# weitong8591/differentiable_ransac

Hardware: AMD Instinct MI355X
Metric: hypotheses/sec (and image-pairs/sec) at 2000 pts x 1024 hyps, 1/2/4/8 GPU (higher is better)
Workload: dtype f32; 1 GPU; nister 5-pt E, 2000 pts x 1024 hyps per pair, Gumbel top-k sampler (in-kernel Philox), MSAC scoring with masks, test mode, 128 pairs/GPU/step; sampler=gumbel, pairs_per_gpu=128, points=2000, hypotheses_per_pair=1024, hypotheses_per_pair_per_gpu=1024, models_per_pair=10240, solver=nister, parallelism=pairs sharded over 1 GPU(s), no collective, streams=1, issue=1 batch(es) in flight, round-robin over 1 HIP stream(s), eager launches

## Files before the change

differentiable_ransac_amd/csrc/dr_common.hpp:

```cpp
#pragma once
#include <hip/hip_runtime.h>
#include <stdint.h>
#include <stdio.h>

#include "../../include/dransac.h"

namespace dr {

constexpr int kWave = 64;

void set_error(const char *fmt, ...);

inline int check_launch(const char *what) {
  hipError_t e = hipGetLastError();
  if (e != hipSuccess) {
    set_error("%s: %s", what, hipGetErrorString(e));
    return DR_ELAUNCH;
  }
  return DR_OK;
}

#define DR_REQUIRE(cond, msg)            \
  do {                                   \
    if (!(cond)) {                       \
      ::dr::set_error("%s: %s", __func__, msg); \
      return DR_EINVAL;                  \
    }                                    \
  } while (0)

struct PairGate {
  const int32_t *iters = nullptr;
  const double *max_iters = nullptr;
  __device__ __forceinline__ bool closed(int p) const { return iters && (double)iters[p] >= max_iters[p]; }
  __device__ __forceinline__ bool closed_range(int first, int last) const {
    if (!iters) return false;
    for (int p = first; p <= last; ++p)
      if (!closed(p)) return false;
    return true;
  }
};

__device__ __forceinline__ void seed_next_block(uint64_t *__restrict__ state, uint64_t *__restrict__ out, int n) {
  const uint64_t s0 = state[0] * 0x9E3779B97F4A7C15ull + state[1];
  for (int i = threadIdx.x; i < n; i += blockDim.x) out[i] = s0 + (uint64_t)i;
  __syncthreads();
  if (threadIdx.x == 0) state[1] += (uint64_t)n;
}

__device__ __forceinline__ void race_weights_block(const float *__restrict__ logits, int N, int P, int p, float *__restrict__ ws) {
  __shared__ float s_mx[4], s_mn[4], s_rate[4];
  __shared__ int s_bad[4];
  const int tid = threadIdx.x, lane = tid & 63, wv = tid >> 6;
  const float *lg = logits + (size_t)p * N;
  constexpr int kRegs = 8;
  const bool in_regs = N <= kRegs * 256;
  float lr[kRegs];
  float mx = -INFINITY, mn = INFINITY;
  int bad = 0;
  if (in_regs) {
#pragma unroll
    for (int u = 0; u < kRegs; ++u) lr[u] = (tid + 256 * u < N) ? lg[tid + 256 * u] : 0.f;
#pragma unroll
    for (int u = 0; u < kRegs; ++u) {
      const bool have = tid + 256 * u < N, fin = fabsf(lr[u]) < INFINITY;
      bad |= (have && !fin) ? 1 : 0;
      mx = (have && fin) ? fmaxf(mx, lr[u]) : mx;
      mn = (have && fin) ? fminf(mn, lr[u]) : mn;
    }
  } else {
    for (int n = tid; n < N; n += 256) {
      const float l = lg[n];
      const bool fin = fabsf(l) < INFINITY;
      bad |= fin ? 0 : 1;
      mx = fin ? fmaxf(mx, l) : mx;
      mn = fin ? fminf(mn, l) : mn;
    }
  }
#pragma unroll
  for (int o = 32; o > 0; o >>= 1) {
    mx = fmaxf(mx, __shfl_xor(mx, o, 64));
    mn = fminf(mn, __shfl_xor(mn, o, 64));
    bad |= __shfl_xor(bad, o, 64);
  }
  if (lane == 0) { s_mx[wv] = mx; s_mn[wv] = mn; s_bad[wv] = bad; }
  __syncthreads();
  mx = fmaxf(fmaxf(s_mx[0], s_mx[1]), fmaxf(s_mx[2], s_mx[3]));
  mn = fminf(fminf(s_mn[0], s_mn[1]), fminf(s_mn[2], s_mn[3]));
  bad = s_bad[0] | s_bad[1] | s_bad[2] | s_bad[3];
  const bool tame = !bad && (mx - mn) <= 80.0f;
  float *w = ws + (size_t)p * N;
  float rate = 0.f;
  if (in_regs) {
#pragma unroll
    for (int u = 0; u < kRegs; ++u) {
      if (tid + 256 * u < N) {
        const float d = (mx - lr[u]) * 1.44269504088896340736f;
        w[tid + 256 * u] = tame ? __builtin_amdgcn_exp2f(d) : 0.f;
        rate += tame ? __builtin_amdgcn_exp2f(-d) : 0.f;
      }
    }
  } else {
    for (int n = tid; n < N; n += 256) {
      const float d = (mx - lg[n]) * 1.44269504088896340736f;
      w[n] = tame ? __builtin_amdgcn_exp2f(d) : 0.f;
      rate += tame ? __builtin_amdgcn_exp2f(-d) : 0.f;
    }
  }
#pragma unroll
  for (int o = 32; o > 0; o >>= 1) rate += __shfl_xor(rate, o, 64);
  if (lane == 0) s_rate[wv] = rate;
  __syncthreads();
  if (tid == 0) {
    reinterpret_cast<int *>(ws + (size_t)P * N)[p] = tame ? 1 : 0;
    ws[(size_t)P * N + P + p] = -1.0f / (0.69314718055994530942f * ((s_rate[0] + s_rate[1]) + (s_rate[2] + s_rate[3])));
    ws[(size_t)P * N + 2 * (size_t)P + p] = mx;
  }
}

template <typename T>
__device__ __forceinline__ T wave_sum(T v) {
#pragma unroll
  for (int o = 32; o > 0; o >>= 1) v += __shfl_xor(v, o, 64);
  return v;
}
__device__ __forceinline__ float wave_sum_lane63(float v) {
  v += __int_as_float(__builtin_amdgcn_mov_dpp(__float_as_int(v), 0xB1, 0xF, 0xF, true));
  v += __int_as_float(__builtin_amdgcn_mov_dpp(__float_as_int(v), 0x4E, 0xF, 0xF, true));
  v += __int_as_float(__builtin_amdgcn_mov_dpp(__float_as_int(v), 0x141, 0xF, 0xF, true));
  v += __int_as_float(__builtin_amdgcn_mov_dpp(__float_as_int(v), 0x140, 0xF, 0xF, true));
  v += __int_as_float(__builtin_amdgcn_update_dpp(0, __float_as_int(v), 0x142, 0xA, 0xF, false));
  v += __int_as_float(__builtin_amdgcn_update_dpp(0, __float_as_int(v), 0x143, 0xC, 0xF, false));
  return v;
}

template <int kCtrl, int kRowMask, bool kBound>
__device__ __forceinline__ double dpp_add_step(double x) {
  const long long xi = __double_as_longlong(x);
  const int lo = (int)xi, hi = (int)(xi >> 32);
  const int tlo = kBound ? __builtin_amdgcn_mov_dpp(lo, kCtrl, kRowMask, 0xF, true) : __builtin_amdgcn_update_dpp(0, lo, kCtrl, kRowMask, 0xF, false);
  const int thi = kBound ? __builtin_amdgcn_mov_dpp(hi, kCtrl, kRowMask, 0xF, true) : __builtin_amdgcn_update_dpp(0, hi, kCtrl, kRowMask, 0xF, false);
  return x + __longlong_as_double(((long long)thi << 32) | (unsigned int)tlo);
}
__device__ __forceinline__ double wave_sum_lane63(double v) {
  v = dpp_add_step<0xB1, 0xF, true>(v);
  v = dpp_add_step<0x4E, 0xF, true>(v);
  v = dpp_add_step<0x141, 0xF, true>(v);
  v = dpp_add_step<0x140, 0xF, true>(v);
  v = dpp_add_step<0x142, 0xA, false>(v);
  v = dpp_add_step<0x143, 0xC, false>(v);
  return v;
}

template <int kCtrl, int kRowMask>
__device__ __forceinline__ float dpp_max_step(float x) {
  const int xi = __float_as_int(x);
  return fmaxf(x, __int_as_float(__builtin_amdgcn_update_dpp(xi, xi, kCtrl, kRowMask, 0xF, false)));
}
__device__ __forceinline__ float wave_max_bcast(float v) {
  v = dpp_max_step<0xB1, 0xF>(v);
  v = dpp_max_step<0x4E, 0xF>(v);
  v = dpp_max_step<0x141, 0xF>(v);
  v = dpp_max_step<0x140, 0xF>(v);
  v = dpp_max_step<0x142, 0xA>(v);
  v = dpp_max_step<0x143, 0xC>(v);
  return __int_as_float(__builtin_amdgcn_readlane(__float_as_int(v), 63));
}
__device__ __forceinline__ float wave_sum_bcast(float v) {
  return __int_as_float(__builtin_amdgcn_readlane(__float_as_int(wave_sum_lane63(v)), 63));
}

template <typename T>
__device__ __forceinline__ T wave_max(T v) {
#pragma unroll
  for (int o = 32; o > 0; o >>= 1) {
    T w = __shfl_xor(v, o, 64);
    v = w > v ? w : v;
  }
  return v;
}

__device__ __forceinline__ float fast_rcp(float x) { return __builtin_amdgcn_rcpf(x); }
__device__ __forceinline__ double fast_rcp(double x) { return 1.0 / x; }

template <typename T>
__device__ __forceinline__ bool is_finite(T x) {
  return __builtin_isfinite(x);
}

struct Philox {
  static constexpr uint32_t M0 = 0xD2511F53u, M1 = 0xCD9E8D57u, W0 = 0x9E3779B9u, W1 = 0xBB67AE85u;
  __host__ __device__ static inline void mulhilo(uint32_t a, uint32_t b, uint32_t &hi, uint32_t &lo) {
    uint64_t p = (uint64_t)a * b;
    hi = (uint32_t)(p >> 32);
    lo = (uint32_t)p;
  }
  __host__ __device__ static inline uint32_t xor3(uint32_t a, uint32_t b, uint32_t c) {
#if defined(__HIP_DEVICE_COMPILE__)
    uint32_t r;
    asm("v_bitop3_b32 %0, %1, %2, %3 bitop3:0x96" : "=v"(r) : "v"(a), "v"(b), "s"(c));
    return r;
#else
    return a ^ b ^ c;
#endif
  }
  __host__ __device__ static inline void gen(uint64_t seed, uint32_t c0, uint32_t c1, uint32_t c2, uint32_t c3,
                                             uint32_t out[4]) {
    uint32_t k0 = (uint32_t)seed, k1 = (uint32_t)(seed >> 32);
    constexpr int kPhiloxRounds = 7;
#pragma unroll
    for (int r = 0; r < kPhiloxRounds; ++r) {
      uint32_t h0, l0, h1, l1;
      mulhilo(M0, c0, h0, l0);
      mulhilo(M1, c2, h1, l1);
      uint32_t n0 = xor3(h1, c1, k0), n1 = l1, n2 = xor3(h0, c3, k1), n3 = l0;
      c0 = n0; c1 = n1; c2 = n2; c3 = n3;
      k0 += W0; k1 += W1;
    }
    out[0] = c0; out[1] = c1; out[2] = c2; out[3] = c3;
  }
};

__device__ __forceinline__ float gumbel_from_bits(uint32_t bits) {
  constexpr float kScale = 2.3283064365386963e-10f * (1.0f - 1.1920928955078125e-07f - 1.17549435e-38f);
  float u = __builtin_fmaf((float)bits, kScale, 1.17549435e-38f);
  const float kLn2 = 0.69314718055994530942f;
  const float t = __builtin_amdgcn_logf(u);
  float g = __builtin_fmaf(-kLn2, __builtin_amdgcn_logf(-t), 0.36651292058166432701f);
  asm("" : "+v"(g));
  return g;
}

#ifdef DR_PROFILE_STAGES
static __device__ unsigned long long g_stage_cycles[32];
#define DR_STAGE_BEGIN() unsigned long long _t_prev = __builtin_readcyclecounter()
#define DR_STAGE(i)                                                        \
  do {                                                                     \
    unsigned long long _t = __builtin_readcyclecounter();                  \
    if ((threadIdx.x & 63) == 0) atomicAdd(&::dr::g_stage_cycles[i], _t - _t_prev); \
    _t_prev = __builtin_readcyclecounter();                                \
  } while (0)
#define DR_DEFINE_STAGE_READER(name)                                                                          \
  extern "C" int name(unsigned long long *out16) {                                            \
    unsigned long long zero[32] = {0};                                                                        \
    if (hipMemcpyFromSymbol(out16, HIP_SYMBOL(::dr::g_stage_cycles), sizeof(zero)) != hipSuccess) return -2; \
    if (hipMemcpyToSymbol(HIP_SYMBOL(::dr::g_stage_cycles), zero, sizeof(zero)) != hipSuccess) return -2;    \
    return 0;                                                                                                 \
  }
#else
#define DR_DEFINE_STAGE_READER(name)
#define DR_STAGE_BEGIN() do {} while (0)
#define DR_STAGE(i) do {} while (0)
#endif

}
```

differentiable_ransac_amd/csrc/gumbel_topk.hip:

```cpp
#include <algorithm>

#include "dr_common.hpp"

namespace dr {

constexpr int kRowsPerBlock = 4;
constexpr int kMaxK = 8;
constexpr int kMaxCand = 64;

template <typename T>
struct GumbelArgs {
  const T *logits;
  const T *gumbel;
  uint64_t seed;
  T tau;
  int P, B, N, k;
  const uint64_t *seed_ptr;
  int sub;
};
__device__ __forceinline__ void sub_batch_row(uint64_t &seed, int &bq, int b, int sub) {
  bq = b;
  if (sub > 0) {
    seed += (uint64_t)(b / sub);
    bq = b % sub;
// ... 204 lines not shown
      if (kSoft) y_sel[row * a.k + pos] = exp_t<T>(mg - wmx) * inv_sm;
      s_win[wv][pos] = me;
    }
  }
  if (kSoft && lane == 0) lse_out[row] = lse;

  if (kSoft && (y_soft || ret)) {
    __builtin_amdgcn_fence(__ATOMIC_ACQ_REL, "workgroup");
    __builtin_amdgcn_wave_barrier();
    int mine[kMaxK];
    for (int r = 0; r < kMaxK; ++r) mine[r] = r < a.k ? winp[r] : -1;
    for (int q = lane; q < groups; q += 64) {
      T g[4];
      if (kCache) {
#pragma unroll
        for (int j = 0; j < 4; ++j) g[j] = gcache[4 * q + j];
      } else {
        T nz[4];
        load_group<T>(a, p, b, q, g, nz);
      }
#pragma unroll
      for (int j = 0; j < 4; ++j) {
        const int n = 4 * q + j;
        if (n >= a.N) continue;
        const T y = exp_t<T>(g[j] - wmx) * inv_sm;
        bool sel = false;
#pragma unroll
        for (int r = 0; r < kMaxK; ++r) sel = sel || (mine[r] == n);
        if (y_soft) y_soft[row * a.N + n] = y;
        if (ret) ret[row * a.N + n] = ((sel ? T(1) : T(0)) - y) + y;
      }
    }
  }
}

__device__ __forceinline__ float log2_uniform_from_bits(uint32_t bits) {
  constexpr float kScale = 2.3283064365386963e-10f * (1.0f - 1.1920928955078125e-07f - 1.17549435e-38f);
  return __builtin_amdgcn_logf(__builtin_fmaf((float)bits, kScale, 1.17549435e-38f));
}

__global__ __launch_bounds__(256) void gumbel_race_weights_kernel(const float *__restrict__ logits, int N, int P, float *__restrict__ ws) {
  race_weights_block(logits, N, P, blockIdx.x, ws);
}

constexpr int kFastGroups = 8;

__device__ __forceinline__ float4 straight_through(float4 m, float y) {
  const float st = (1.0f - y) + y;
  return make_float4(m.x * st, m.y * st, m.z * st, m.w * st);
}

template <bool kSoft, bool kScreen = false>
__global__ __launch_bounds__(kRowsPerBlock * 64) void gumbel_topk_fast_kernel(const float *__restrict__ logits, uint64_t seed,
                                                                             int B, int N, int k, int32_t *__restrict__ idx,
                                                                             float *__restrict__ y_sel,
                                                                             float *__restrict__ lse_out,
                                                                             const uint64_t *__restrict__ seed_ptr,
                                                                             const float4 *__restrict__ gather_src = nullptr,
                                                                             float4 *__restrict__ gather_dst = nullptr,
                                                                             PairGate gate = PairGate(),
                                                                             const uint32_t *__restrict__ screen_tb = nullptr,
                                                                             const float *__restrict__ screen_T = nullptr,
                                                                             int sub = 0, const float *__restrict__ race_ws = nullptr,
                                                                             int P_race = 0) {
  if (gate.closed(blockIdx.y)) return;
  static_assert(!(kSoft && kScreen), "the soft-max statistics need every element's score");
  __shared__ float s_val[kRowsPerBlock][kMaxCand];
  __shared__ int s_idx[kRowsPerBlock][kMaxCand];
  if (seed_ptr) seed = *seed_ptr;
  const int lane = threadIdx.x & 63;
  int wv = threadIdx.x >> 6;
  wv = __builtin_amdgcn_readfirstlane(wv);
  const int p = blockIdx.y, b = blockIdx.x * kRowsPerBlock + wv;
  if (b >= B) return;
  int bq;
  sub_batch_row(seed, bq, b, sub);
  const int groups = N >> 2;
  const size_t row = (size_t)p * B + b;
  const float4 *lg = reinterpret_cast<const float4 *>(logits + (size_t)p * N);
  float *cand_val = s_val[wv];
  int *cand_idx = s_idx[wv];

  if constexpr (kScreen) {
    const float Tf = screen_T[p];
    if (Tf != INFINITY) {
      const uint4 *tb4 = reinterpret_cast<const uint4 *>(screen_tb + (size_t)p * N);
      int ncand = 0, reach = 0;
      uint4 t_nx = lane < groups ? tb4[lane] : make_uint4(0xffffffffu, 0xffffffffu, 0xffffffffu, 0xffffffffu);
      float4 l_nx = lane < groups ? lg[lane] : make_float4(0.f, 0.f, 0.f, 0.f);
#pragma unroll
      for (int i = 0; i < kFastGroups; ++i) {
        if (64 * i >= groups) break;
        const int q = lane + 64 * i;
        const bool inb = q < groups;
        const uint4 t4 = t_nx;
        const float4 l4v = l_nx;
        if (i + 1 < kFastGroups) {
          const int qn = q + 64;
          t_nx = qn < groups ? tb4[qn] : make_uint4(0xffffffffu, 0xffffffffu, 0xffffffffu, 0xffffffffu);
          l_nx = qn < groups ? lg[qn] : make_float4(0.f, 0.f, 0.f, 0.f);
        }
        uint32_t r[4];
        Philox::gen(seed, (uint32_t)q, (uint32_t)bq, (uint32_t)p, 0u, r);
        const uint32_t tt[4] = {t4.x, t4.y, t4.z, t4.w};
        const float ll[4] = {l4v.x, l4v.y, l4v.z, l4v.w};
#pragma unroll
        for (int j = 0; j < 4; ++j) {
          const bool has = inb && r[j] >= tt[j];
          const unsigned long long bal = __builtin_amdgcn_ballot_w64(has);
          if (bal) {
            float gv = -INFINITY;
            if (has) {
              gv = ll[j] + gumbel_from_bits(r[j]);
              const int pos = ncand + __popcll(bal & ((1ull << lane) - 1ull));
              if (pos < kMaxCand) { cand_val[pos] = gv; cand_idx[pos] = 4 * q + j; }
            }
            ncand += __popcll(bal);
            reach += __popcll(__builtin_amdgcn_ballot_w64(has && gv >= Tf));
          }
        }
      }
      __builtin_amdgcn_fence(__ATOMIC_ACQ_REL, "workgroup");
      __builtin_amdgcn_wave_barrier();
      if (reach >= k && ncand <= kMaxCand) {
        const bool have = lane < ncand;
        const float cv = have ? cand_val[lane] : -INFINITY;
        const int ci = have ? cand_idx[lane] : 0x7fffffff;
        int rank = 0;
        for (int j = 0; j < ncand; ++j) {
          const float ov = cand_val[j];
          const int oi = cand_idx[j];
          rank += (ov > cv) || (ov == cv && oi < ci);
        }
        const bool win = have && rank < k;
        const unsigned long long wb = __ballot(win);
        int pos = 0;
        for (int j = 0; j < ncand; ++j) {
          if ((wb >> j) & 1ull) pos += cand_idx[j] < ci;
        }
        if (win) {
          idx[row * k + pos] = ci;
          if (gather_dst) gather_dst[row * k + pos] = gather_src[(size_t)p * N + ci];
        }
        return;
      }
      __builtin_amdgcn_wave_barrier();
    }
  }

  float g[kFastGroups][4];
  float mx = -INFINITY, sm = 0.f, lmax = -INFINITY;
  bool race = false;
  if constexpr (!kScreen) race = race_ws != nullptr && reinterpret_cast<const int *>(race_ws + (size_t)P_race * N)[p] != 0;
  if (race) {
    const float4 *wr = reinterpret_cast<const float4 *>(race_ws + (size_t)p * N);
#pragma unroll
    for (int i = 0; i < kFastGroups; ++i) {
      const int q = lane + 64 * i;
      if (q < groups) {
        uint32_t r[4];
        Philox::gen(seed, (uint32_t)q, (uint32_t)bq, (uint32_t)p, 0u, r);
        const float4 w4 = wr[q];
        g[i][0] = w4.x * log2_uniform_from_bits(r[0]);
        g[i][1] = w4.y * log2_uniform_from_bits(r[1]);
        g[i][2] = w4.z * log2_uniform_from_bits(r[2]);
        g[i][3] = w4.w * log2_uniform_from_bits(r[3]);
        lmax = fmaxf(lmax, fmaxf(fmaxf(g[i][0], g[i][1]), fmaxf(g[i][2], g[i][3])));
        if (kSoft) sm += (__builtin_amdgcn_rcpf(-g[i][0]) + __builtin_amdgcn_rcpf(-g[i][1])) +
                         (__builtin_amdgcn_rcpf(-g[i][2]) + __builtin_amdgcn_rcpf(-g[i][3]));
      } else {
#pragma unroll
        for (int j = 0; j < 4; ++j) g[i][j] = -INFINITY;
      }
    }
  } else
#pragma unroll
  for (int i = 0; i < kFastGroups; ++i) {
    const int q = lane + 64 * i;
    if (q < groups) {
      uint32_t r[4];
      Philox::gen(seed, (uint32_t)q, (uint32_t)bq, (uint32_t)p, 0u, r);
      const float4 l = lg[q];
      g[i][0] = l.x + gumbel_from_bits(r[0]);
      g[i][1] = l.y + gumbel_from_bits(r[1]);
      g[i][2] = l.z + gumbel_from_bits(r[2]);
      g[i][3] = l.w + gumbel_from_bits(r[3]);
      const float gm = fmaxf(fmaxf(g[i][0], g[i][1]), fmaxf(g[i][2], g[i][3]));
      lmax = fmaxf(lmax, gm);
      if (kSoft) {
        if (gm > mx) { sm *= exp_t<float>(mx - gm); mx = gm; }
#pragma unroll
        for (int j = 0; j < 4; ++j) sm += exp_t<float>(g[i][j] - mx);
      }
    } else {
#pragma unroll
      for (int j = 0; j < 4; ++j) g[i][j] = -INFINITY;
    }
  }
  float wmx = 0.f, lse = 0.f, inv_sm = 0.f;
  if (kSoft) {
    if (race) {
      sm = row_sum(sm);
      lse = race_ws[(size_t)P_race * N + 2 * (size_t)P_race + p] + (log_t<float>(sm) + 0.36651292058166432701f);
      inv_sm = 1.0f / sm;
    } else {
      wmx = row_max(mx);
      sm *= (mx == -INFINITY) ? 0.f : exp_t<float>(mx - wmx);
      sm = row_sum(sm);
      lse = wmx + log_t<float>(sm);
      inv_sm = 1.0f / sm;
    }
  }
  auto y_of = [&](float score) { return race ? __builtin_amdgcn_rcpf(-score) * inv_sm : exp_t<float>(score - wmx) * inv_sm; };

  bool settled = false;
  float thr = -INFINITY;
  if constexpr (!kScreen) if (race) {
    const float inv = race_ws[(size_t)P_race * N + P_race + p];
    const float kf = (float)k + 0.5f;
    float t = 6.0f * inv, tlo = 0.f, thi = 0.f;
    int clo = 0;
    bool have_lo = false, have_hi = false;
#pragma unroll
    for (int it = 0; it < 6; ++it) {
      const int c = __popcll(__builtin_amdgcn_ballot_w64(lmax >= t));
      if (c >= k) { tlo = t; clo = c; have_lo = true; if (c == k) break; }
      else { thi = t; have_hi = true; }
      t = (have_lo && have_hi) ? 0.5f * (tlo + thi) : t * fminf(4.0f, kf * __builtin_amdgcn_rcpf((float)c + 0.5f));
    }
    if (have_lo && clo <= 16) { settled = true; thr = tlo; }
  }
  if (!settled) {
    float v = lmax;
    for (int r = 0; r < k; ++r) {
      thr = row_max(v);
      const unsigned long long who = __ballot(v == thr);
      if (lane == __ffsll((long long)who) - 1) v = -INFINITY;
    }
  }

  if constexpr (!kScreen) {
    int n = 0;
    int cv_i = __float_as_int(-INFINITY), ci = 0x7fffffff;
#pragma unroll
    for (int i = 0; i < kFastGroups; ++i) {
      if (64 * i >= groups) break;
      const unsigned long long c0 = __builtin_amdgcn_ballot_w64(g[i][0] >= thr), c1 = __builtin_amdgcn_ballot_w64(g[i][1] >= thr),
                               c2 = __builtin_amdgcn_ballot_w64(g[i][2] >= thr), c3 = __builtin_amdgcn_ballot_w64(g[i][3] >= thr);
      unsigned long long any = c0 | c1 | c2 | c3;
      while (any) {
        const int l = __builtin_ctzll(any);
        any &= any - 1;
        const unsigned long long cj[4] = {c0, c1, c2, c3};
#pragma unroll
        for (int j = 0; j < 4; ++j) {
          if ((cj[j] >> l) & 1ull) {
            const bool mine = __builtin_amdgcn_inverse_ballot_w64(1ull << (n & 63));
            cv_i = mine ? __builtin_amdgcn_readlane(__float_as_int(g[i][j]), l) : cv_i;
            ci = mine ? 4 * (l + 64 * i) + j : ci;
            ++n;
          }
        }
      }
    }
    if (n <= 64) {
      const float cv = __int_as_float(cv_i);
      bool win = lane < n;
      int pos = lane;
      if (n > k) {
        int rank = 0;
#pragma unroll 1
        for (int m = 0; m < n; ++m) {
          const float ov = __int_as_float(__builtin_amdgcn_readlane(cv_i, m));
          const int oi = __builtin_amdgcn_readlane(ci, m);
          rank += (ov > cv) || (ov == cv && oi < ci);
        }
        win = win && rank < k;
        pos = __popcll(__builtin_amdgcn_ballot_w64(win) & ((1ull << lane) - 1ull));
      }
      if (win) {
        idx[row * k + pos] = ci;
        if (kSoft) {
          const float y = y_of(cv);
          y_sel[row * k + pos] = y;
          if (gather_dst) gather_dst[row * k + pos] = straight_through(gather_src[(size_t)p * N + ci], y);
        }
        if (!kSoft && gather_dst) gather_dst[row * k + pos] = gather_src[(size_t)p * N + ci];
      }
      if (kSoft && lane == 0) lse_out[row] = lse;
      return;
    }
    if (settled) {
      float v = lmax;
      for (int r = 0; r < k; ++r) {
        thr = row_max(v);
        const unsigned long long who = __ballot(v == thr);
        if (lane == __ffsll((long long)who) - 1) v = -INFINITY;
      }
    }
  }

  int ncand = 0;
#pragma unroll
  for (int i = 0; i < kFastGroups; ++i) {
    if (64 * i >= groups) break;
    const int q = lane + 64 * i;
    if (!__ballot(fmaxf(fmaxf(g[i][0], g[i][1]), fmaxf(g[i][2], g[i][3])) >= thr)) continue;
#pragma unroll
    for (int j = 0; j < 4; ++j) {
      const bool c = g[i][j] >= thr;
      const unsigned long long bal = __ballot(c);
      if (bal) {
        const int pos = ncand + __popcll(bal & ((1ull << lane) - 1ull));
        if (c && pos < kMaxCand) { cand_val[pos] = g[i][j]; cand_idx[pos] = 4 * q + j; }
        ncand += __popcll(bal);
      }
    }
  }
  __builtin_amdgcn_fence(__ATOMIC_ACQ_REL, "workgroup");
  __builtin_amdgcn_wave_barrier();

  if (ncand <= kMaxCand) {
    const bool have = lane < ncand;
    const float cv = have ? cand_val[lane] : -INFINITY;
    const int ci = have ? cand_idx[lane] : 0x7fffffff;
    int rank = 0;
    for (int j = 0; j < ncand; ++j) {
      const float ov = cand_val[j];
      const int oi = cand_idx[j];
      rank += (ov > cv) || (ov == cv && oi < ci);
    }
    const bool win = have && rank < k;
    const unsigned long long wb = __ballot(win);
    int pos = 0;
    for (int j = 0; j < ncand; ++j) {
      if ((wb >> j) & 1ull) pos += cand_idx[j] < ci;
    }
    if (win) {
      idx[row * k + pos] = ci;
      if (kSoft) {
        const float y = y_of(cv);
        y_sel[row * k + pos] = y;
        if (gather_dst) gather_dst[row * k + pos] = straight_through(gather_src[(size_t)p * N + ci], y);
      }
      if (!kSoft && gather_dst) gather_dst[row * k + pos] = gather_src[(size_t)p * N + ci];
    }
  } else {
    int won[kMaxK];
    float wong[kMaxK];
    for (int r = 0; r < k; ++r) {
      float bv = -INFINITY;
      int bi = 0x7fffffff;
#pragma unroll
      for (int i = 0; i < kFastGroups; ++i) {
#pragma unroll
        for (int j = 0; j < 4; ++j) {
          const int n = 4 * (lane + 64 * i) + j;
          bool skip = n >= N;
          for (int s = 0; s < r; ++s) skip = skip || (won[s] == n);
          if (!skip && (g[i][j] > bv || (g[i][j] == bv && n < bi))) { bv = g[i][j]; bi = n; }
        }
      }
#pragma unroll
      for (int o = 32; o > 0; o >>= 1) {
        const float ov = __shfl_xor(bv, o, 64);
        const int oi = __shfl_xor(bi, o, 64);
        if (ov > bv || (ov == bv && oi < bi)) { bv = ov; bi = oi; }
      }
      won[r] = bi;
      wong[r] = bv;
// ... 918 lines not shown
```

differentiable_ransac_amd/ops.py:

```python
from __future__ import annotations

import os as _os
from typing import Optional, Tuple

import torch

from . import _lib as L
from ._lib import c_int, c_uint64, ptr, stream

SCREEN_SHORT_ROWS = _os.environ.get("DRANSAC_SCREEN_SHORT", "0") == "1"


K1_RACE = _os.environ.get("DRANSAC_K1_RACE", "1") != "0"
K1_RACE_SOFT = _os.environ.get("DRANSAC_K1_RACE_SOFT", "1") != "0"
_RACE_MIN = tuple(int(v) for v in _os.environ.get("DRANSAC_K1_RACE_MIN", "32768,32").split(","))
FUSED_SAMPLE_GATHER = _os.environ.get("DRANSAC_FUSED_SAMPLE_GATHER", "1") != "0"
FUSED_MATCH_LOSS = True


def _u8(t: Optional[torch.Tensor]) -> Optional[torch.Tensor]:
    return None if t is None else t.contiguous().view(torch.uint8)


def _u8_ptr(t: Optional[torch.Tensor]):
    return ptr(_u8(t))


def _gate_args(gate):
    return (ptr(None), ptr(None)) if gate is None else (ptr(gate.iters), ptr(gate.max_iters))


def _dev_seed(seed):
    if torch.is_tensor(seed):
        if seed.dtype != torch.int64 or seed.numel() != 1 or not seed.is_cuda:
            L._reset()
            raise L.DransacError("a device seed is a one-element int64 CUDA tensor (DeviceSeed.next())")
        return True
    return False


def _seed_args(seed):
    if _dev_seed(seed):
        return c_uint64(0), ptr(seed)
    return c_uint64(seed & (2 ** 64 - 1)), ptr(None)


def _thr_tensor(threshold, P: int, like: torch.Tensor) -> torch.Tensor:
    if isinstance(threshold, torch.Tensor):
        t = threshold.to(device=like.device, dtype=like.dtype).reshape(-1)
        if t.numel() == 1 and P > 1:
            t = t.expand(P)
        return t.contiguous()
    return torch.full((P,), float(threshold), device=like.device, dtype=like.dtype)


def msac_score(matches: torch.Tensor, models: torch.Tensor, threshold, want_masks: bool = True,
               valid: Optional[torch.Tensor] = None, path: int = 0, gate=None) -> Tuple[torch.Tensor, Optional[torch.Tensor]]:
    P, N, _ = matches.shape
    M = models.shape[1]
    matches = matches.contiguous()
    models = models.contiguous()
    thr = _thr_tensor(threshold, P, matches)
    scores = torch.empty((P, M), device=matches.device, dtype=matches.dtype)
    masks = torch.empty((P, M, N), device=matches.device, dtype=torch.bool) if want_masks else None
    v = _u8(valid)
    if path not in (0, 1):
        raise L.DransacError("msac_score: path must be 0 or 1 (the general kernels); path 2, the matrix-core candidate filter of "
                             "round 2, was measured slower and left the library (scratch/k4_filter_kernel.patch)")
    if matches.dtype == torch.float32:
        L.call("dr_msac_score_f32", ptr(matches), ptr(models), ptr(v), ptr(thr), c_int(P), c_int(M), c_int(N), ptr(scores),
               ptr(masks), *_gate_args(gate), stream())
        return scores, masks
    L.call(f"dr_msac_score_{L.suffix(matches.dtype)}", ptr(matches), ptr(models), ptr(v), ptr(thr), c_int(P), c_int(M), c_int(N),
           ptr(scores), ptr(masks), stream())
    return scores, masks


def select_best(matches: torch.Tensor, models: torch.Tensor, scores: torch.Tensor, threshold,
                valid: Optional[torch.Tensor] = None):
    P, N, _ = matches.shape
    M = models.shape[1]
    dev, dt = matches.device, matches.dtype
    thr = _thr_tensor(threshold, P, matches)
    best_idx = torch.empty((P,), device=dev, dtype=torch.int32)
    best_score = torch.empty((P,), device=dev, dtype=dt)
    best_model = torch.empty((P, 3, 3), device=dev, dtype=dt)
    best_mask = torch.empty((P, N), device=dev, dtype=torch.bool)
    inliers = torch.empty((P,), device=dev, dtype=torch.int32)
    L.call(f"dr_select_best_{L.suffix(dt)}", ptr(matches.contiguous()), ptr(models.contiguous()), _u8_ptr(valid),
           ptr(scores.contiguous()), ptr(thr), c_int(P), c_int(M), c_int(N), ptr(best_idx), ptr(best_score),
           ptr(best_model), ptr(best_mask), ptr(inliers), stream())
    return best_idx, best_score, best_model, best_mask, inliers


class RansacState:

    def __init__(self, P: int, N: int, max_iterations: int, device, dtype, _init: bool = True, packed: bool = False):
        alloc = torch.zeros if _init else torch.empty
        self.packed = None
        if packed and P == 1 and dtype == torch.float32 and not _init:
            self.packed = torch.empty(44 + N, device=device, dtype=torch.uint8)
            self.best_model = self.packed[:36].view(torch.float32).view(1, 3, 3)
            self.best_score = self.packed[36:40].view(torch.float32)
            self.iters = self.packed[40:44].view(torch.int32)
            self.best_mask = self.packed[44:].view(torch.bool).view(1, N)
        else:
            self.best_score = alloc(P, device=device, dtype=dtype)
            self.best_model = (torch.eye(3, device=device, dtype=dtype).repeat(P, 1, 1) if _init
                               else torch.empty(P, 3, 3, device=device, dtype=dtype))
            self.best_mask = alloc(P, N, device=device, dtype=torch.bool)
            self.iters = alloc(P, device=device, dtype=torch.int32)
        self.best_inliers = alloc(P, device=device, dtype=torch.int32)
        self.max_iters = (torch.full((P,), float(max_iterations), device=device, dtype=torch.float64) if _init
                          else torch.empty(P, device=device, dtype=torch.float64))
        self.max_iterations = max_iterations


def ransac_init(P: int, N: int, max_iterations: int, threshold: float, K1: Optional[torch.Tensor],
                K2: Optional[torch.Tensor], device, dtype, seeds=None, packed: bool = False,
                race_logits: Optional[torch.Tensor] = None) -> Tuple[RansacState, torch.Tensor]:
    st = RansacState(P, N, max_iterations, device, dtype, _init=False, packed=packed)
    st.seeds = None
    st.race_ws = None
    if race_logits is not None:
        if race_logits.dtype != torch.float32 or race_logits.shape != (P, N) or not race_logits.is_contiguous():
            raise L.DransacError("ransac_init: race_logits must be contiguous f32 [P,N]")
        st.race_ws = torch.empty((P, N + 32), device=device, dtype=torch.float32)
    seed_state = None
    n_seeds = 0
    if seeds is not None:
        seed_state, n_seeds = seeds[0].state, int(seeds[1])
        st.seeds = torch.empty(n_seeds, dtype=torch.int64, device=device)
    thr = torch.empty(P, device=device, dtype=dtype)
    k_stride = 0
    if K1 is not None:
        K1 = K1.to(device=device, dtype=dtype).contiguous()
        K2 = K2.to(device=device, dtype=dtype).contiguous()
        if K1.dim() == 3 and K1.shape[0] != 1:
            if K1.shape[0] != P or K2.shape != K1.shape:
                raise ValueError("K1/K2 must be [3,3] or [P,3,3]")
            k_stride = 9
    L.call(f"dr_ransac_init_{L.suffix(dtype)}", ptr(K1), ptr(K2), c_int(k_stride), L.c_double(float(threshold)),
           c_int(P), c_int(N), c_int(max_iterations), ptr(thr), ptr(st.best_score), ptr(st.best_model),
           ptr(st.best_mask), ptr(st.best_inliers), ptr(st.iters), ptr(st.max_iters), ptr(seed_state), ptr(st.seeds),
           c_int(n_seeds), ptr(race_logits), ptr(st.race_ws), stream())
    return st, thr


def ransac_update(state: RansacState, matches, models, valid, scores, thr, B: int, k: int, confidence: float = 0.999,
                  eps: float = 1e-5, sub_models: int = 0) -> None:
    P, N, _ = matches.shape
    M = models.shape[1]
    if sub_models and M > sub_models * 512:
        raise L.DransacError("ransac_update: at most 512 sub-batches per launch")
    L.call(f"dr_ransac_update_{L.suffix(matches.dtype)}", ptr(matches), ptr(models.contiguous()), _u8_ptr(valid),
           ptr(scores.contiguous()), ptr(thr), c_int(P), c_int(M), c_int(N), c_int(B), c_int(k),
           L.c_double(confidence), L.c_double(eps), c_int(state.max_iterations), ptr(state.best_score),
           ptr(state.best_model), ptr(state.best_mask), ptr(state.best_inliers), ptr(state.iters), ptr(state.max_iters),
           c_int(int(sub_models)), stream())


def local_optimize(state: RansacState, matches, thr, fundamental: bool, lo: int, lo_iters: int, k: int,
                   confidence: float = 0.999, eps: float = 1e-5, max_iterations: Optional[int] = None,
                   lo_seen: Optional[torch.Tensor] = None, lo_refits: Optional[torch.Tensor] = None) -> None:
    tensors = (matches, thr, lo_seen, lo_refits, state.best_score, state.best_model, state.best_mask, state.best_inliers,
               state.max_iters)
    if any(t is not None and not t.is_cuda for t in tensors):
        raise L.DransacError("libdransac operates on GPU tensors only (got a CPU tensor)")
    P, N, _ = matches.shape
    if lo_seen is None or lo_seen.shape != (P, 10) or lo_seen.dtype != matches.dtype or not lo_seen.is_contiguous():
        raise L.DransacError("local_optimize: lo_seen must be a contiguous [P,10] tensor of the matches' dtype")
    if lo_refits is not None and (lo_refits.shape != (P,) or lo_refits.dtype != torch.int32):
        raise L.DransacError("local_optimize: lo_refits must be [P] int32")
    mi = state.max_iterations if max_iterations is None else max_iterations
    L.call(f"dr_local_opt_{L.suffix(matches.dtype)}", ptr(matches.contiguous()), ptr(thr), c_int(P), c_int(N),
           c_int(1 if fundamental else 0), c_int(int(lo)), c_int(int(lo_iters)), c_int(int(k)), L.c_double(confidence),
           L.c_double(eps), c_int(int(mi)), ptr(state.best_score), ptr(state.best_model), ptr(state.best_mask.view(torch.uint8)),
           ptr(state.best_inliers), ptr(state.max_iters), ptr(lo_seen), ptr(lo_refits), stream())


class DeviceSeed:

    def __init__(self, base: int, device, calls: int = 0):
        def signed(v):
            v &= 2 ** 64 - 1
            return v - 2 ** 64 if v >= 2 ** 63 else v
        self.state = torch.tensor([signed(base), signed(calls)], dtype=torch.int64, device=device)

    def next(self) -> torch.Tensor:
        out = torch.empty(1, dtype=torch.int64, device=self.state.device)
        L.call("dr_seed_next_n", ptr(self.state), ptr(out), c_int(1), stream())
        return out

    def next_block(self, n: int) -> torch.Tensor:
        out = torch.empty(n, dtype=torch.int64, device=self.state.device)
        L.call("dr_seed_next_n", ptr(self.state), ptr(out), c_int(n), stream())
        return out

    def next_n(self, n: int):
        out = self.next_block(n)
        return [out[i:i + 1] for i in range(n)]


def gumbel_topk(logits: Optional[torch.Tensor], B: int, k: int, tau: float = 1.0,
                gumbel: Optional[torch.Tensor] = None, seed: int = 0, N: Optional[int] = None,
                dense: bool = False, want_noise: bool = False, device=None, dtype=torch.float32, soft: bool = True,
                screen: Optional[bool] = None):
    if not soft and dense:
        raise ValueError("the dense outputs need the soft-max statistics (soft=True)")
    if logits is not None:
        logits = logits.contiguous()
        P, N = logits.shape
        device, dtype = logits.device, logits.dtype
    else:
        P = 1 if gumbel is None else gumbel.shape[0]
        assert N is not None and device is not None
    if gumbel is not None:
        gumbel = gumbel.contiguous()
        assert gumbel.shape == (P, B, N) and gumbel.dtype == dtype
    idx = torch.empty((P, B, k), device=device, dtype=torch.int32)
    if (not soft and logits is not None and gumbel is None and not want_noise and dtype == torch.float32 and tau == 1.0
            and N > 2048 and N % 4 == 0 and k <= 5 and (B >= 64 if screen is None else screen)):
        ws = torch.empty(((N + 32) * P,), device=device, dtype=torch.int32)
        L.call("dr_gumbel_topk_index_f32", ptr(logits), *_seed_args(seed), L.c_float(tau), c_int(P), c_int(B), c_int(N), c_int(k),
               ptr(idx), ptr(ws), stream())
        return dict(idx=idx, y_sel=None, lse=None)
    y_sel = torch.empty((P, B, k), device=device, dtype=dtype) if soft else None
    lse = torch.empty((P, B), device=device, dtype=dtype) if soft else None
    y_soft = torch.empty((P, B, N), device=device, dtype=dtype) if dense else None
    ret = torch.empty((P, B, N), device=device, dtype=dtype) if dense else None
    noise = torch.empty((P, B, N), device=device, dtype=dtype) if want_noise else None
    if _dev_seed(seed) and (gumbel is not None or dense or want_noise or logits is None):
        raise L.DransacError("a device seed serves the in-kernel noise of given logits only (no explicit noise / dense outputs)")
    L.call(f"dr_gumbel_topk_fwd_{L.suffix(dtype)}", ptr(logits), ptr(gumbel), *_seed_args(seed), L.scalar(dtype, tau), c_int(P),
           c_int(B), c_int(N), c_int(k), ptr(idx), ptr(y_sel), ptr(lse), ptr(y_soft), ptr(ret), ptr(noise), stream())
    out = dict(idx=idx, y_sel=y_sel, lse=lse)
    if dense:
        out.update(y_soft=y_soft, ret=ret)
    if want_noise:
        out["gumbel"] = noise
    return out


def race_form_pays(P: int, B: int, N: int, tau: float) -> bool:
    return K1_RACE and P * B >= _RACE_MIN[0] and P >= _RACE_MIN[1] and N <= 2048 and N % 4 == 0 and tau == 1.0


def gumbel_topk_gather(matches: torch.Tensor, logits: torch.Tensor, B: int, k: int, tau: float = 1.0, seed=0, gate=None,
                       screen: Optional[bool] = None, sub: int = 0, race: Optional[bool] = None, race_ws: Optional[torch.Tensor] = None):
    if matches.dtype != torch.float32 or logits.dtype != torch.float32 or matches.shape[-1] != 4:
        raise L.DransacError("gumbel_topk_gather: f32 two-view correspondences [P,N,4]")
    matches, logits = matches.contiguous(), logits.contiguous()
    P, N = logits.shape
    idx = torch.empty((P, B, k), device=logits.device, dtype=torch.int32)
    samples = torch.empty((P, B, k, 4), device=logits.device, dtype=torch.float32)
    want_screen = SCREEN_SHORT_ROWS if screen is None else screen
    ws = (torch.empty((P, N + 32), device=logits.device, dtype=torch.int32)
          if want_screen and N <= 2048 and N % 4 == 0 and tau == 1.0 and k <= 5 and B >= 64 else None)
    ready = race_ws is not None and ws is None and N <= 2048 and N % 4 == 0 and tau == 1.0
    want_race = not ready and (race_form_pays(P, B, N, tau) if race is None else race) and ws is None and N <= 2048 and N % 4 == 0 and tau == 1.0
    rws = race_ws if ready else (torch.empty((P, N + 32), device=logits.device, dtype=torch.float32) if want_race else None)
    L.call("dr_gumbel_topk_gather_f32", ptr(logits), ptr(matches), *_seed_args(seed), L.c_float(tau), c_int(P), c_int(B), c_int(N),
           c_int(k), ptr(idx), ptr(samples), ptr(ws), *_gate_args(gate), c_int(0 if sub >= B else int(sub)), ptr(rws),
           c_int(1 if ready else 0), stream())
    return idx, samples


def gumbel_topk_bwd(logits, gumbel, seed, tau, idx, lse, a_sel):
    P, B, k = idx.shape
    N = logits.shape[1]
    grad = torch.empty_like(logits)
    if logits.dtype == torch.float64:
        if _dev_seed(seed):
            raise L.DransacError("gumbel_topk_bwd: device seeds serve f32 only")
        L.call("dr_gumbel_topk_bwd_f64", ptr(logits.contiguous()), ptr(gumbel), c_uint64(seed & (2 ** 64 - 1)),
               L.c_double(tau), c_int(P), c_int(B), c_int(N), c_int(k), ptr(idx), ptr(lse.contiguous()),
               ptr(a_sel.to(torch.float64).contiguous()), ptr(grad), stream())
        return grad
    L.call("dr_gumbel_topk_bwd_f32", ptr(logits.contiguous()), ptr(None if _dev_seed(seed) else gumbel), *_seed_args(seed),
           L.c_float(tau), c_int(P), c_int(B), c_int(N), c_int(k), ptr(idx), ptr(lse), ptr(a_sel.contiguous()), ptr(grad), stream())
    return grad


def topdown_sample(logits: Optional[torch.Tensor], B: int, k: int, seed: int = 0, N: Optional[int] = None, P: int = 1,
                   device=None) -> torch.Tensor:
    if logits is not None:
        logits = logits.contiguous()
        P, N = logits.shape
        device = logits.device
        sfx = L.suffix(logits.dtype)
    else:
        sfx = "f32"
    ws = torch.empty((P, N), device=device, dtype=torch.float64)
    idx = torch.empty((P, B, k), device=device, dtype=torch.int32)
    if sfx == "f32":
        L.call("dr_topdown_sample_f32", ptr(logits), *_seed_args(seed), c_int(P), c_int(B), c_int(N), c_int(k), ptr(ws), ptr(idx),
               stream())
        return idx
    if _dev_seed(seed):
        raise L.DransacError("device seeds: f32 logits")
    L.call("dr_topdown_sample_f64", ptr(logits), _seed_args(seed)[0], c_int(P), c_int(B), c_int(N), c_int(k), ptr(ws), ptr(idx),
           stream())
    return idx


def uniform_sample(P: int, B: int, k: int, N: int, seed: int, device) -> torch.Tensor:
    idx = torch.empty((P, B, k), device=device, dtype=torch.int32)
    L.call("dr_uniform_sample", *_seed_args(seed), c_int(P), c_int(B), c_int(k), c_int(N), ptr(idx), stream())
    return idx


def gather(matches: torch.Tensor, idx: torch.Tensor, y_sel: Optional[torch.Tensor] = None) -> torch.Tensor:
    P, N, c = matches.shape
    _, B, k = idx.shape
    out = torch.empty((P, B, k, c), device=matches.device, dtype=matches.dtype)
    L.call(f"dr_gather_fwd_{L.suffix(matches.dtype)}", ptr(matches.contiguous()), ptr(idx), ptr(y_sel), c_int(P),
           c_int(N), c_int(B), c_int(k), c_int(c), ptr(out), stream())
    return out


def gather_bwd(matches, idx, y_sel, grad_samples, grad_w=None, want_grad_matches=False):
    P, N, c = matches.shape
    _, B, k = idx.shape
    a_sel = torch.empty((P, B, k), device=matches.device, dtype=matches.dtype)
    gm = torch.zeros_like(matches) if want_grad_matches else None
    dt = matches.dtype
    L.call(f"dr_gather_bwd_{L.suffix(dt)}", ptr(matches.contiguous()), ptr(idx), ptr(y_sel), ptr(grad_samples.to(dt).contiguous()),
           ptr(None if grad_w is None else grad_w.to(dt).contiguous()), c_int(P), c_int(N), c_int(B), c_int(k), c_int(c),
           ptr(a_sel), ptr(gm), stream())
    return a_sel, gm


class SampleGather(torch.autograd.Function):

    @staticmethod
    def forward(ctx, matches, logits, B, k, tau, gumbel, seed):
        ctx.set_materialize_grads(False)
        if logits.dtype == torch.float64 and logits.requires_grad and gumbel is None and _dev_seed(seed):
            raise L.DransacError("SampleGather: f64 logits with a device seed have no backward (device seeds serve f32 only)")
        fused = (FUSED_SAMPLE_GATHER and gumbel is None and logits.dtype == torch.float32 and matches.dtype == torch.float32
                 and matches.shape[-1] == 4)
        if fused:
            matches, logits = matches.contiguous(), logits.contiguous()
            P, N = logits.shape
            r = dict(idx=torch.empty((P, B, k), device=logits.device, dtype=torch.int32),
                     y_sel=torch.empty((P, B, k), device=logits.device, dtype=torch.float32),
                     lse=torch.empty((P, B), device=logits.device, dtype=torch.float32))
            samples = torch.empty((P, B, k, 4), device=logits.device, dtype=torch.float32)
            rws = (torch.empty((P, N + 32), device=logits.device, dtype=torch.float32)
                   if K1_RACE_SOFT and race_form_pays(P, B, N, tau) else None)
            L.call("dr_gumbel_topk_gather_soft_f32", ptr(logits), ptr(matches), *_seed_args(seed), L.c_float(tau), c_int(P), c_int(B),
                   c_int(N), c_int(k), ptr(r["idx"]), ptr(r["y_sel"]), ptr(r["lse"]), ptr(samples), ptr(rws), stream())
        else:
            r = gumbel_topk(logits, B, k, tau, gumbel, seed)
            samples = gather(matches, r["idx"], r["y_sel"])
        ctx.save_for_backward(matches, logits, r["idx"], r["y_sel"], r["lse"], gumbel if gumbel is not None else
                              torch.empty(0, device=logits.device))
        ctx.cfg = (tau, seed, gumbel is not None)
        ctx.fused = fused
        ctx.mark_non_differentiable(r["idx"])
        return samples, r["y_sel"], r["idx"]

    @staticmethod
    def backward(ctx, g_samples, g_w, _g_idx):
        if g_samples is None and g_w is None:
            return (None,) * 7
        matches, logits, idx, y_sel, lse, gumbel = ctx.saved_tensors
        if g_samples is None:
            g_samples = torch.zeros(idx.shape + (matches.shape[-1],), device=matches.device, dtype=matches.dtype)
        tau, seed, has_noise = ctx.cfg
        if ctx.fused and not ctx.needs_input_grad[0]:
            P, B, k = idx.shape
            gl = torch.empty_like(logits)
            L.call("dr_gumbel_topk_gather_bwd_f32", ptr(logits), ptr(matches), *_seed_args(seed), L.c_float(tau), c_int(P), c_int(B),
                   c_int(logits.shape[1]), c_int(k), ptr(idx), ptr(lse), ptr(g_samples.contiguous()),
                   ptr(None if g_w is None else g_w.contiguous()), ptr(gl), stream())
            return None, gl, None, None, None, None, None
        a_sel, gm = gather_bwd(matches, idx, y_sel, g_samples, g_w, want_grad_matches=ctx.needs_input_grad[0])
        gl = gumbel_topk_bwd(logits, gumbel if has_noise else None, seed, tau, idx, lse, a_sel)
        return gm, gl, None, None, None, None, None


def _flat_samples(samples: torch.Tensor, c: int):
    s = samples.reshape(-1, samples.shape[-2], c).contiguous()
    return s, s.shape[0], s.shape[1]


def _solver_gate(gate, s: torch.Tensor, n: int):
    if gate is None:
        return 0, None
    if n != 5 or s.dtype != torch.float32:
        raise L.DransacError("the gated five-point entries take f32 minimal samples")
    return int(gate[1]), gate[0]


def solve_nister5(samples: torch.Tensor, weights: Optional[torch.Tensor] = None, path: int = 0, gate=None):
    s, Bt, n = _flat_samples(samples, 4)
    lead = samples.shape[:-2]
    models = torch.empty((Bt, 10, 3, 3), device=s.device, dtype=s.dtype)
    valid = torch.empty((Bt, 10), device=s.device, dtype=torch.bool)
    w = None if weights is None else weights.reshape(Bt, n).to(s.dtype).contiguous()
    if path != 0 and (n != 5 or s.dtype != torch.float32):
        raise L.DransacError("an explicit five-point kernel path exists for f32 minimal samples only")
    rows, st = _solver_gate(gate, s, n)
    if s.dtype == torch.float32:
        L.call("dr_solve_nister5_f32", ptr(s), ptr(w), c_int(Bt), c_int(n), ptr(models), ptr(None), ptr(valid), c_int(path), c_int(rows),
               *_gate_args(st), stream())
    else:
        L.call(f"dr_solve_nister5_{L.suffix(s.dtype)}", ptr(s), ptr(w), c_int(Bt), c_int(n), ptr(models), ptr(valid), stream())
    return models.reshape(*lead, 10, 3, 3), valid.reshape(*lead, 10)


def solve_nister5_hp(samples: torch.Tensor, weights: Optional[torch.Tensor] = None, path: int = 0):
    s, Bt, n = _flat_samples(samples, 4)
    if n != 5 or s.dtype != torch.float32:
        raise L.DransacError("solve_nister5_hp takes f32 minimal samples (5 correspondences)")
    lead = samples.shape[:-2]
    models = torch.empty((Bt, 10, 3, 3), device=s.device, dtype=torch.float32)
    m64 = torch.empty((Bt, 10, 3, 3), device=s.device, dtype=torch.float64)
    valid = torch.empty((Bt, 10), device=s.device, dtype=torch.bool)
    w = None if weights is None else weights.reshape(Bt, n).to(s.dtype).contiguous()
    L.call("dr_solve_nister5_f32", ptr(s), ptr(w), c_int(Bt), c_int(5), ptr(models), ptr(m64), ptr(valid), c_int(path), c_int(0),
           ptr(None), ptr(None), stream())
    return models.reshape(*lead, 10, 3, 3), m64.reshape(*lead, 10, 3, 3), valid.reshape(*lead, 10)


def solve_essential_gated(samples: torch.Tensor, which: str, gate):
    return (solve_nister5 if which == "nister" else solve_stewenius5)(samples, gate=(gate, samples.shape[1]))


def debug_real_roots10(coef: torch.Tensor, method: int = 1):
    coef = coef.to(torch.float64).contiguous()
    n = coef.shape[0]
    roots = torch.zeros((n, 2, 10), device=coef.device, dtype=torch.float64)
    counts = torch.zeros((n, 2), device=coef.device, dtype=torch.int32)
    L.call("dr_debug_real_roots10", ptr(coef), c_int(n), c_int(method), ptr(roots), ptr(counts), stream())
    return roots, counts


def solve_stewenius5(samples: torch.Tensor, path: int = 0, gate=None):
    s, Bt, n = _flat_samples(samples, 4)
    if n != 5:
        raise L.DransacError("the Stewenius solver takes exactly 5 correspondences per sample")
    lead = samples.shape[:-2]
    models = torch.empty((Bt, 10, 3, 3), device=s.device, dtype=s.dtype)
    valid = torch.empty((Bt, 10), device=s.device, dtype=torch.bool)
    if path != 0 and s.dtype != torch.float32:
        raise L.DransacError("an explicit five-point kernel path exists for f32 minimal samples only")
    rows, st = _solver_gate(gate, s, n)
    if s.dtype == torch.float32:
        L.call("dr_solve_stewenius5_f32", ptr(s), c_int(Bt), ptr(models), ptr(valid), c_int(path), c_int(rows), *_gate_args(st), stream())
    else:
        L.call(f"dr_solve_stewenius5_{L.suffix(s.dtype)}", ptr(s), c_int(Bt), ptr(models), ptr(valid), stream())
    return models.reshape(*lead, 10, 3, 3), valid.reshape(*lead, 10)


def solve_f8(samples: torch.Tensor, weights: Optional[torch.Tensor] = None):
    s, Bt, n = _flat_samples(samples, 4)
    lead = samples.shape[:-2]
    models = torch.empty((Bt, 3, 3), device=s.device, dtype=s.dtype)
    valid = torch.empty((Bt,), device=s.device, dtype=torch.bool)
    w = None if weights is None else weights.reshape(Bt, n).to(s.dtype).contiguous()
    L.call(f"dr_solve_f8_{L.suffix(s.dtype)}", ptr(s), ptr(w), c_int(Bt), c_int(n), ptr(models), ptr(valid), stream())
    return models.reshape(*lead, 3, 3), valid.reshape(lead)


def solve_f8_uniform(matches: torch.Tensor, B: int, seed):
    if matches.dtype != torch.float32 or matches.shape[-1] != 4:
        raise L.DransacError("solve_f8_uniform: f32 correspondences [P,N,4]")
    P, N, _ = matches.shape
    idx = torch.empty((P, B, 8), device=matches.device, dtype=torch.int32)
    models = torch.empty((P, B, 3, 3), device=matches.device, dtype=torch.float32)
    valid = torch.empty((P, B), device=matches.device, dtype=torch.bool)
    L.call("dr_solve_f8_uniform_f32", ptr(matches.contiguous()), *_seed_args(seed), c_int(P), c_int(B), c_int(N), ptr(idx),
           ptr(models), ptr(valid), stream())
    return idx, models, valid


def solve_f7(samples: torch.Tensor):
    s, Bt, n = _flat_samples(samples, 4)
    if n != 7:
        raise L.DransacError("the 7-point solver takes exactly 7 correspondences per sample")
    lead = samples.shape[:-2]
    models = torch.empty((Bt, 4, 3, 3), device=s.device, dtype=s.dtype)
    valid = torch.empty((Bt, 4), device=s.device, dtype=torch.bool)
    L.call(f"dr_solve_f7_{L.suffix(s.dtype)}", ptr(s), c_int(Bt), ptr(models), ptr(valid), stream())
    return models.reshape(*lead, 4, 3, 3), valid.reshape(*lead, 4)


def solve_rigid(samples: torch.Tensor, weights: Optional[torch.Tensor] = None, flag: bool = True):
    s, Bt, n = _flat_samples(samples, 6)
    lead = samples.shape[:-2]
    dev, dt = s.device, s.dtype
    model = torch.empty((Bt, 4, 4), device=dev, dtype=dt)
    R = torch.empty((Bt, 3, 3), device=dev, dtype=dt)
    t = torch.empty((Bt, 3), device=dev, dtype=dt)
    scale = torch.empty((Bt,), device=dev, dtype=dt)
    valid = torch.empty((Bt,), device=dev, dtype=torch.bool)
    w = None if weights is None else weights.reshape(Bt, n).to(dt).contiguous()
    L.call(f"dr_solve_rigid_{L.suffix(dt)}", ptr(s), ptr(w), c_int(Bt), c_int(n), c_int(1 if flag else 0), ptr(model),
           ptr(R), ptr(t), ptr(scale), ptr(valid), stream())
    return (model.reshape(*lead, 4, 4), R.reshape(*lead, 3, 3), t.reshape(*lead, 3), scale.reshape(lead),
# ... 584 lines not shown
```

Measured before the change: 142.4 million hypotheses/s.

## Screen Gumbel race candidates with precomputed integer word thresholds

Precomputes a per-point uint32 threshold on raw Philox words so the hard top-k race path can select candidates by integer comparison, without computing log-uniform keys for every point. Candidates from ballots are compacted into lanes, and only those get exact keys and a rank-based top-k. A fallback runs when fewer than k candidates pass or more than 64 do. The race workspace doubles in size and the weights kernel does extra work per point. The old bisection threshold search is now limited to the soft path.

Measured after the change: 138.5 million hypotheses/s. 2.8% lower.

```diff
diff --git a/differentiable_ransac_amd/csrc/dr_common.hpp b/differentiable_ransac_amd/csrc/dr_common.hpp
--- a/differentiable_ransac_amd/csrc/dr_common.hpp
+++ b/differentiable_ransac_amd/csrc/dr_common.hpp
@@ -47,6 +47,7 @@
   if (threadIdx.x == 0) state[1] += (uint64_t)n;
 }
 
+constexpr float kRaceLambda = 16.0f;
 __device__ __forceinline__ void race_weights_block(const float *__restrict__ logits, int N, int P, int p, float *__restrict__ ws) {
   __shared__ float s_mx[4], s_mn[4], s_rate[4];
   __shared__ int s_bad[4];
@@ -110,10 +111,29 @@
   for (int o = 32; o > 0; o >>= 1) rate += __shfl_xor(rate, o, 64);
   if (lane == 0) s_rate[wv] = rate;
   __syncthreads();
+  const float inv = -1.0f / (0.69314718055994530942f * ((s_rate[0] + s_rate[1]) + (s_rate[2] + s_rate[3])));
+  const float t = kRaceLambda * inv;
   if (tid == 0) {
     reinterpret_cast<int *>(ws + (size_t)P * N)[p] = tame ? 1 : 0;
-    ws[(size_t)P * N + P + p] = -1.0f / (0.69314718055994530942f * ((s_rate[0] + s_rate[1]) + (s_rate[2] + s_rate[3])));
+    ws[(size_t)P * N + P + p] = inv;
     ws[(size_t)P * N + 2 * (size_t)P + p] = mx;
+    ws[(size_t)P * N + 3 * (size_t)P + p] = t;
+  }
+  uint32_t *tw = reinterpret_cast<uint32_t *>(ws + (size_t)P * (N + 32)) + (size_t)p * N;
+  auto word_threshold = [&](float wn) {
+    const float x = (t * __builtin_amdgcn_rcpf(wn)) * (1.0f + 1.9073486328125e-06f);
+    return (uint32_t)((__builtin_amdgcn_exp2f(x) * 4294967296.0f) * (1.0f - 9.5367431640625e-07f));
+  };
+  if (in_regs) {
+#pragma unroll
+    for (int u = 0; u < kRegs; ++u) {
+      if (tid + 256 * u < N) {
+        const float d = (mx - lr[u]) * 1.44269504088896340736f;
+        tw[tid + 256 * u] = tame ? word_threshold(__builtin_amdgcn_exp2f(d)) : 0u;
+      }
+    }
+  } else {
+    for (int n = tid; n < N; n += 256) tw[n] = tame ? word_threshold(w[n]) : 0u;
   }
 }
 
diff --git a/differentiable_ransac_amd/csrc/gumbel_topk.hip b/differentiable_ransac_amd/csrc/gumbel_topk.hip
--- a/differentiable_ransac_amd/csrc/gumbel_topk.hip
+++ b/differentiable_ransac_amd/csrc/gumbel_topk.hip
@@ -380,6 +380,64 @@
   float mx = -INFINITY, sm = 0.f, lmax = -INFINITY;
   bool race = false;
   if constexpr (!kScreen) race = race_ws != nullptr && reinterpret_cast<const int *>(race_ws + (size_t)P_race * N)[p] != 0;
+  if constexpr (!kSoft && !kScreen) if (race) {
+    const uint4 *tw4 = reinterpret_cast<const uint4 *>(race_ws + (size_t)P_race * (N + 32)) + (size_t)p * groups;
+    const float t = race_ws[(size_t)P_race * N + 3 * (size_t)P_race + p];
+    int n = 0;
+    int cw = 0, ci = 0;
+    uint4 t_nx = lane < groups ? tw4[lane] : make_uint4(0xffffffffu, 0xffffffffu, 0xffffffffu, 0xffffffffu);
+#pragma unroll
+    for (int i = 0; i < kFastGroups; ++i) {
+      if (64 * i >= groups) break;
+      const int q = lane + 64 * i;
+      const bool inb = q < groups;
+      const uint4 t4 = t_nx;
+      if (i + 1 < kFastGroups) {
+        const int qn = q + 64;
+        t_nx = qn < groups ? tw4[qn] : make_uint4(0xffffffffu, 0xffffffffu, 0xffffffffu, 0xffffffffu);
+      }
+      uint32_t r[4];
+      Philox::gen(seed, (uint32_t)q, (uint32_t)bq, (uint32_t)p, 0u, r);
+      const unsigned long long c0 = __builtin_amdgcn_ballot_w64(inb && r[0] >= t4.x), c1 = __builtin_amdgcn_ballot_w64(inb && r[1] >= t4.y),
+                               c2 = __builtin_amdgcn_ballot_w64(inb && r[2] >= t4.z), c3 = __builtin_amdgcn_ballot_w64(inb && r[3] >= t4.w);
+      unsigned long long any = c0 | c1 | c2 | c3;
+      while (any) {
+        const int l = __builtin_ctzll(any);
+        any &= any - 1;
+        const unsigned long long cj[4] = {c0, c1, c2, c3};
+#pragma unroll
+        for (int j = 0; j < 4; ++j) {
+          if ((cj[j] >> l) & 1ull) {
+            const bool mine = __builtin_amdgcn_inverse_ballot_w64(1ull << (n & 63));
+            cw = mine ? __builtin_amdgcn_readlane((int)r[j], l) : cw;
+            ci = mine ? 4 * (l + 64 * i) + j : ci;
+            ++n;
+          }
+        }
+      }
+    }
+    if (n <= 64) {
+      const bool have = lane < n;
+      const float cv = have ? race_ws[(size_t)p * N + ci] * log2_uniform_from_bits((uint32_t)cw) : -INFINITY;
+      const int cv_i = __float_as_int(cv);
+      if (__popcll(__builtin_amdgcn_ballot_w64(cv >= t)) >= k) {
+        int rank = 0;
+#pragma unroll 1
+        for (int m = 0; m < n; ++m) {
+          const float ov = __int_as_float(__builtin_amdgcn_readlane(cv_i, m));
+          const int oi = __builtin_amdgcn_readlane(ci, m);
+          rank += (ov > cv) || (ov == cv && oi < ci);
+        }
+        const bool win = have && rank < k;
+        const int pos = __popcll(__builtin_amdgcn_ballot_w64(win) & ((1ull << lane) - 1ull));
+        if (win) {
+          idx[row * k + pos] = ci;
+          if (gather_dst) gather_dst[row * k + pos] = gather_src[(size_t)p * N + ci];
+        }
+        return;
+      }
+    }
+  }
   if (race) {
     const float4 *wr = reinterpret_cast<const float4 *>(race_ws + (size_t)p * N);
 #pragma unroll
@@ -443,7 +501,7 @@
 
   bool settled = false;
   float thr = -INFINITY;
-  if constexpr (!kScreen) if (race) {
+  if constexpr (kSoft) if (race) {
     const float inv = race_ws[(size_t)P_race * N + P_race + p];
     const float kf = (float)k + 0.5f;
     float t = 6.0f * inv, tlo = 0.f, thi = 0.f;
diff --git a/differentiable_ransac_amd/ops.py b/differentiable_ransac_amd/ops.py
--- a/differentiable_ransac_amd/ops.py
+++ b/differentiable_ransac_amd/ops.py
@@ -125,7 +125,7 @@
     if race_logits is not None:
         if race_logits.dtype != torch.float32 or race_logits.shape != (P, N) or not race_logits.is_contiguous():
             raise L.DransacError("ransac_init: race_logits must be contiguous f32 [P,N]")
-        st.race_ws = torch.empty((P, N + 32), device=device, dtype=torch.float32)
+        st.race_ws = torch.empty((P, 2 * N + 32), device=device, dtype=torch.float32)
     seed_state = None
     n_seeds = 0
     if seeds is not None:
@@ -259,7 +259,7 @@
           if want_screen and N <= 2048 and N % 4 == 0 and tau == 1.0 and k <= 5 and B >= 64 else None)
     ready = race_ws is not None and ws is None and N <= 2048 and N % 4 == 0 and tau == 1.0
     want_race = not ready and (race_form_pays(P, B, N, tau) if race is None else race) and ws is None and N <= 2048 and N % 4 == 0 and tau == 1.0
-    rws = race_ws if ready else (torch.empty((P, N + 32), device=logits.device, dtype=torch.float32) if want_race else None)
+    rws = race_ws if ready else (torch.empty((P, 2 * N + 32), device=logits.device, dtype=torch.float32) if want_race else None)
     L.call("dr_gumbel_topk_gather_f32", ptr(logits), ptr(matches), *_seed_args(seed), L.c_float(tau), c_int(P), c_int(B), c_int(N),
            c_int(k), ptr(idx), ptr(samples), ptr(ws), *_gate_args(gate), c_int(0 if sub >= B else int(sub)), ptr(rws),
            c_int(1 if ready else 0), stream())
@@ -347,7 +347,7 @@
                      y_sel=torch.empty((P, B, k), device=logits.device, dtype=torch.float32),
                      lse=torch.empty((P, B), device=logits.device, dtype=torch.float32))
             samples = torch.empty((P, B, k, 4), device=logits.device, dtype=torch.float32)
-            rws = (torch.empty((P, N + 32), device=logits.device, dtype=torch.float32)
+            rws = (torch.empty((P, 2 * N + 32), device=logits.device, dtype=torch.float32)
                    if K1_RACE_SOFT and race_form_pays(P, B, N, tau) else None)
             L.call("dr_gumbel_topk_gather_soft_f32", ptr(logits), ptr(matches), *_seed_args(seed), L.c_float(tau), c_int(P), c_int(B),
                    c_int(N), c_int(k), ptr(r["idx"]), ptr(r["y_sel"]), ptr(r["lse"]), ptr(samples), ptr(rws), stream())
diff --git a/scratch/sim_k1_word_screen.py b/scratch/sim_k1_word_screen.py
--- /dev/null
+++ b/scratch/sim_k1_word_screen.py
@@ -0,0 +1,43 @@
+import os, sys
+import numpy as np
+ROOT = os.path.dirname(os.path.dirname(os.path.abspath(__file__)))
+sys.path.insert(0, ROOT); sys.path.insert(0, os.path.join(ROOT, "tests"))
+import philox_ref
+from differentiable_ransac_amd import synth
+
+def exact_share(q, k):
+    f = np.zeros(k); f[0] = 1.0
+    for x in q:
+        f[1:] = f[1:] * (1 - x) + f[:-1] * x
+        f[0] *= (1 - x)
+    return f.sum()
+
+def run(name, logits, k, lam, B=256, seed=1234):
+    P, N = logits.shape
+    lg = logits.astype(np.float64)
+    w = np.exp(lg.max(1, keepdims=True) - lg)
+    cp = np.log(2) * (1 / w).sum(1)
+    t = -lam / cp
+    q = 1 - np.exp2(t[:, None] / w)
+    ex = np.array([exact_share(q[p], k) for p in range(P)])
+    qi = np.arange(N // 4, dtype=np.uint32)[None, None, :]
+    fb = rows = 0; cnt = []
+    for p0 in range(0, P, 16):
+        pp = np.arange(p0, min(P, p0 + 16), dtype=np.uint32)[:, None, None]
+        b = np.arange(B, dtype=np.uint32)[None, :, None]
+        wd = np.stack(philox_ref.philox4x32(seed, qi, b, pp, np.uint32(0)), -1).reshape(len(pp), B, N)
+        u = wd.astype(np.float32).astype(np.float64) * 2.0 ** -32 + 1.17549435e-38
+        key = w[p0:p0 + 16, None, :] * np.log2(u)
+        c = (key >= t[p0:p0 + 16, None, None]).sum(-1)
+        fb += int(((c < k) | (c > 64)).sum()); rows += c.size; cnt.append(c.ravel())
+    cnt = np.concatenate(cnt)
+    print(f"{name:10s} k={k} lambda={lam:4.1f}: exact P(count<k) mean {ex.mean():.2e} worst pair {ex.max():.2e} | observed {fb}/{rows} = {fb / rows:.2e}"
+          f" | candidates mean {cnt.mean():.2f} p99 {np.percentile(cnt, 99):.0f} max {cnt.max()}")
+
+if __name__ == "__main__":
+    syn = synth.batch_two_view(128, 2000, seed0=0)["logits"].numpy()
+    z = np.load(os.path.join(ROOT, "tests", "golden", "clnet_logits.npz"))
+    cl = z["log_probs"]
+    for lam in (14.0, 16.0, 18.0, 20.0):
+        run("synthetic", syn, 5, lam)
+        run("clnet", cl, 5, lam)
```
